# qinliuliuqin/Medical-Segmentation3d-Toolkit

Measured on AMD Instinct MI355X. Metric: patches/sec (96^3, 1-mod V-Net) train-step, higher is better.
Workload: dtype f32; 1 GPU; vnet(1,2) train step (fwd + Dice loss + bwd + fused Adam), 4 patches of 96^3 per GPU, fp32, random-init weights; global_batch=4, patch=96, parallelism=single GPU, wgrad_overlap=True, train_step_hipgraph=False, step_mode=auto, full=False

## Files before the change

### include/seg3d_hip.h

```cpp
#ifndef SEG3D_HIP_H
#define SEG3D_HIP_H

#ifdef __cplusplus
extern "C" {
#endif

#define SEG3D_ABI_VERSION 2

const char* seg3d_last_error(void);
int seg3d_abi_version(void);
const char* seg3d_target_arch(void);
int seg3d_device_count(void);

int seg3d_ncdhw_to_ndhwc(const float* in, float* out, int N, int C, long long S, void* stream);
int seg3d_ndhwc_to_ncdhw(const float* in, float* out, int N, int C, long long S, void* stream);
int seg3d_copy_channels(const float* src, float* dst, long long nvox, int C, int src_ld, int src_off, int dst_ld,
                        int dst_off, void* stream);

int seg3d_pack_weights_tapmajor(const float* w, float* wp, int A, int B, int BP, int T, long long sa, long long sb,
                                int flip, void* stream);
int seg3d_pack_weights_mfma(const float* w, float* wp, int A, int B, int T, long long sa, long long sb, int flip,
                            void* stream);
long long seg3d_packed_mfma_floats(int A, int B, int T);
typedef struct Seg3dPackJob {
// ... 41 lines not shown
int seg3d_bf16_to_f32(const void* src_bf16, float* dst, long long n, void* stream);
int seg3d_conv3d_k3_wino_supported(int N, int D, int H, int W, int Cin, int Cout);
int seg3d_conv3d_k3_wino_preferred(int N, int D, int H, int W, int Cin, int Cout);
long long seg3d_conv3d_k3_wino_stats_count(int N, int D, int H, int W, int Cin, int Cout);
int seg3d_conv3d_k3_wino_fwd(const float* x, const float* wp_wino, const float* bias, const float* addend, float* y,
                             float* stats_partial, int N, int D, int H, int W, int Cin, int Cout, void* stream);
int seg3d_conv3d_k3_wino2d_supported(int N, int D, int H, int W, int Cin, int Cout);
int seg3d_conv3d_k3_wino2d_preferred(int N, int D, int H, int W, int Cin, int Cout);
long long seg3d_conv3d_k3_wino2d_stats_count(int N, int D, int H, int W, int Cin, int Cout);
int seg3d_conv3d_k3_wino2d_fwd(const float* x, const float* wp_wino2d, const float* bias, const float* addend, float* y,
                               float* stats_partial, int N, int D, int H, int W, int Cin, int Cout, void* stream);
long long seg3d_conv3d_k3_wino2d_fwd_workspace_floats(int N, int D, int H, int W, int Cin, int Cout);
int seg3d_conv3d_k3_wino2d_fwd_ws(const float* x, const float* wp_wino2d, const float* bias, const float* addend, float* y,
                                  float* stats_partial, float* workspace, int N, int D, int H, int W, int Cin, int Cout,
                                  void* stream);
int seg3d_conv3d_k3_wino_wgrad_supported(int N, int D, int H, int W, int Cin, int Cout);
long long seg3d_conv3d_k3_wino_wgrad_workspace_floats(int N, int D, int H, int W, int Cin, int Cout);
int seg3d_conv3d_k3_wino_wgrad(const float* x, const float* dy, float* dw, float* workspace, int N, int D, int H, int W,
                               int Cin, int Cout, int accumulate, void* stream);
int seg3d_conv3d_k3_wino2d_wgrad_supported(int N, int D, int H, int W, int Cin, int Cout);
int seg3d_conv3d_k3_wino2d_wgrad_preferred(int N, int D, int H, int W, int Cin, int Cout);
long long seg3d_conv3d_k3_wino2d_wgrad_workspace_floats(int N, int D, int H, int W, int Cin, int Cout);
int seg3d_conv3d_k3_wino2d_wgrad(const float* x, const float* dy, float* dw, float* workspace, int N, int D, int H, int W,
                                 int Cin, int Cout, int accumulate, void* stream);
int seg3d_conv3d_k3_wino2d_fwd_variant(int N, int D, int H, int W, int Cin, int Cout);
int seg3d_conv3d_k3_wino2d_fwd_sk_chunks(int N, int D, int H, int W, int Cin, int Cout);
int seg3d_conv3d_k3_wino_wgrad_variant(int N, int D, int H, int W, int Cin, int Cout);
int seg3d_conv3d_k3_wino2d_wgrad_variant(int N, int D, int H, int W, int Cin, int Cout);
long long seg3d_conv3d_k3_bf16_stats_count(int N, int D, int H, int W, int Cin, int Cout);
long long seg3d_conv3d_k3_bf16_fwd_workspace_floats(int N, int D, int H, int W, int Cin, int Cout);
// ... 381 lines not shown
```

### medical-segmentation3d-toolkit_amd/csrc/conv_wino2d.hip

```cpp
#include "seg3d_common.h"
#include <type_traits>
#include <utility>
#include "seg3d_hip.h"
#include <stdint.h>

typedef float f32x16 __attribute__((ext_vector_type(16)));
typedef float f32x4 __attribute__((ext_vector_type(4)));
typedef float f32x2 __attribute__((ext_vector_type(2)));

#define W2_TS 8
#define W2_H (W2_TS + 2)
#define W2_NV (W2_H * W2_H * W2_H)
#define W2_NQ 16
#define W2_RAW 4096
#define W2_T (16 * W2_H * W2_NQ * 4)
#define W2_W (48 * 128)
#define W2_LDS_FLOATS (2 * W2_RAW + 2 * W2_T + 2 * W2_W)

__device__ __attribute__((aligned(16))) float w2_zero16[4];

typedef __attribute__((address_space(3))) float w2_lds_float;
__device__ __forceinline__ void w2_glds16(const float* src, float* lds_dst_wave_uniform) {
  const unsigned off = __builtin_amdgcn_readfirstlane((unsigned)(uintptr_t)(w2_lds_float*)lds_dst_wave_uniform);
  asm volatile("s_mov_b32 m0, %1\n\ts_nop 0\n\tglobal_load_lds_dwordx4 %0, off" : : "v"(src), "s"(off) : "memory", "m0");
// ... 96 lines not shown
  float bs[16];
#pragma unroll
  for (int r = 0; r < 16; ++r) bs[r] = __int_as_float(__builtin_amdgcn_readfirstlane(__float_as_int(bias[ub + r])));
  f32x4 b4;
#pragma unroll
  for (int r = 0; r < 4; ++r) b4[r] = kq == 0 ? bs[r] : (kq == 1 ? bs[4 + r] : (kq == 2 ? bs[8 + r] : bs[12 + r]));
  return b4;
}

template <bool BIAS, bool ADD>
__global__ __launch_bounds__(512, 1) void conv3d_k3_wino2d_kernel(const float* __restrict__ x, const float* __restrict__ wp,
                                                                      const float* __restrict__ bias, float* __restrict__ y,
                                                                      float* __restrict__ stats, int N, int D, int H, int W,
                                                                      int Cin, int Cout, int ntz, int nty, int ntx, int ncog,
                                                                      int nitems, const float* __restrict__ addend, int sk_per,
                                                                      float* __restrict__ skws) {
  extern __shared__ __attribute__((aligned(16))) float lds[];
  float* raw = lds;
  float* timg = lds + 2 * W2_RAW;
  float* wbuf = lds + 2 * W2_RAW + 2 * W2_T;
  const int tid = threadIdx.x;
  const int lane = tid & 63;
  const int wave = __builtin_amdgcn_readfirstlane(tid >> 6);
  const int zw = wave & 3, hh = wave >> 2;
  const int l16 = lane & 15, kq = lane >> 4;
  const int NSC = Cin >> 2;
  const int AB = Cin >> 3;
  const int G = gridDim.x;
  auto fdiv = [](int v, float r) { return (int)(((float)v + 0.5f) * r); };
  const float rNTX = 1.0f / (float)ntx, rNTY = 1.0f / (float)nty, rNTZ = 1.0f / (float)ntz, rNCOG = 1.0f / (float)ncog;

// ... 276 lines not shown
      ++gchunk;
#endif
    }

    int co_lane = cur_cog * 32 + 16 * hh + 4 * kq;
    int vo_q = quad_voxel(cur_n, cur_z0, cur_y0, cur_x0);
    const int stat_slot = (cur_n * (ntz * nty * ntx) + cur_tile) * ncog + cur_cog;
    const bool piece = sc_b > 0 || sc_e < NSC;
    float* obase = y;
    int oHW = H * W, oW = W, oC = Cout;
    if (piece) {
      obase = skws + (i64)(2 * sk_wg + (sc_b > 0 ? 0 : 1)) * (W2_TS * W2_TS * W2_TS * 32);
      oHW = W2_TS * W2_TS, oW = W2_TS, oC = 32;
      vo_q = ((2 * zw) * W2_TS + 2 * (l16 >> 2)) * W2_TS + 2 * (l16 & 3);
      co_lane = 16 * hh + 4 * kq;
    }
    int nco_lane = co_lane, nvo_q = vo_q;
    if (more_items) {
      decode(next_item, cur_n, cur_z0, cur_y0, cur_x0, cur_cog, cur_tile);
      nco_lane = cur_cog * 32 + 16 * hh + 4 * kq;
      nvo_q = quad_voxel(cur_n, cur_z0, cur_y0, cur_x0);
    }
    f32x2 s0p = {0.f, 0.f}, s1p = {0.f, 0.f};
    f32x2 v[2][2][2][2];
    auto out_transform = [&](int zz) __attribute__((always_inline)) {
#pragma unroll
      for (int h2 = 0; h2 < 2; ++h2) {
        f32x2 r0[4], r1[4];
#pragma unroll
        for (int px = 0; px < 4; ++px) {
          const f32x2 m0 = {acc[px][zz][2 * h2], acc[px][zz][2 * h2 + 1]}, m1 = {acc[4 + px][zz][2 * h2], acc[4 + px][zz][2 * h2 + 1]};
          const f32x2 m2 = {acc[8 + px][zz][2 * h2], acc[8 + px][zz][2 * h2 + 1]}, m3 = {acc[12 + px][zz][2 * h2], acc[12 + px][zz][2 * h2 + 1]};
// ... 453 lines not shown
}
extern "C" long long seg3d_conv3d_k3_wino2d_fwd_workspace_floats(int N, int D, int H, int W, int Cin, int Cout) {
  if (!seg3d_conv3d_k3_wino2d_supported(N, D, H, W, Cin, Cout)) return 0;
  return w2_sk_per(N, D, H, W, Cin, Cout) > 0 ? 2ll * seg3d_device_cus() * (W2_TS * W2_TS * W2_TS * 32) : 0;
}

extern "C" int seg3d_conv3d_k3_wino2d_fwd_variant(int N, int D, int H, int W, int Cin, int Cout) {
  if (!seg3d_conv3d_k3_wino2d_supported(N, D, H, W, Cin, Cout)) return 0;
  return w2_tiles(D, H, W) ? W2_TS : w2_cells_per_item(N, D, H, W, Cout);
}
extern "C" int seg3d_conv3d_k3_wino2d_fwd_sk_chunks(int N, int D, int H, int W, int Cin, int Cout) {
  if (!seg3d_conv3d_k3_wino2d_supported(N, D, H, W, Cin, Cout)) return 0;
  return w2_sk_per(N, D, H, W, Cin, Cout);
}

extern "C" int seg3d_conv3d_k3_wino2d_fwd_ws(const float* x, const float* wp, const float* bias, const float* addend, float* y,
                                             float* stats, float* workspace, int N, int D, int H, int W, int Cin, int Cout,
                                             void* stream) {
  SEG3D_REQUIRE(x && wp && y, "seg3d_conv3d_k3_wino2d_fwd: null pointer");
  SEG3D_REQUIRE(seg3d_conv3d_k3_wino2d_supported(N, D, H, W, Cin, Cout),
                "seg3d_conv3d_k3_wino2d_fwd: shape not supported (whole 4^3 cells, Cin %% 8 == 0, Cout %% 32 == 0)");
  const int ncog = Cout / 32;
  const int nitems = (int)w2_items(N, D, H, W, Cout);
  const int sk_per = workspace ? w2_sk_per(N, D, H, W, Cin, Cout) : 0;
  dim3 grid(sk_per > 0 ? (unsigned)seg3d_device_cus() : seg3d_persistent_grid(nitems), 1, 1);
  if (w2_tiles(D, H, W)) {
    static Seg3dOncePerDevice configured[4];
    if (int rc = seg3d_allow_full_lds(reinterpret_cast<const void*>(&conv3d_k3_wino2d_kernel<false, false>), configured[0], "conv3d_k3_wino2d")) return rc;
    if (int rc = seg3d_allow_full_lds(reinterpret_cast<const void*>(&conv3d_k3_wino2d_kernel<true, false>), configured[1], "conv3d_k3_wino2d")) return rc;
    if (int rc = seg3d_allow_full_lds(reinterpret_cast<const void*>(&conv3d_k3_wino2d_kernel<false, true>), configured[2], "conv3d_k3_wino2d")) return rc;
    if (int rc = seg3d_allow_full_lds(reinterpret_cast<const void*>(&conv3d_k3_wino2d_kernel<true, true>), configured[3], "conv3d_k3_wino2d")) return rc;
    const int ntz = D / W2_TS, nty = H / W2_TS, ntx = W / W2_TS;
#define W2_LAUNCH(B_, A_)                                                                                                       \
  hipLaunchKernelGGL((conv3d_k3_wino2d_kernel<B_, A_>), grid, dim3(64 * W2_NW), (size_t)W2_LDS_FLOATS * 4, (hipStream_t)stream, x, \
                     wp, bias, y, stats, N, D, H, W, Cin, Cout, ntz, nty, ntx, ncog, nitems, addend, sk_per, workspace)
    if (bias) {
      if (addend) W2_LAUNCH(true, true); else W2_LAUNCH(true, false);
    } else {
      if (addend) W2_LAUNCH(false, true); else W2_LAUNCH(false, false);
    }
#undef W2_LAUNCH
    if (sk_per > 0) {
      SEG3D_LAUNCH_CHECK("seg3d_conv3d_k3_wino2d_fwd");
      hipLaunchKernelGGL(conv3d_k3_wino2d_sk_finish_kernel, dim3(grid.x - 1), dim3(512), 0, (hipStream_t)stream, workspace, y, stats, D,
                         H, W, Cout, ntz, nty, ntx, ncog, nitems, Cin / 4, sk_per);
    }
  } else {
    static Seg3dOncePerDevice configured[8];
    if (int rc = seg3d_allow_full_lds(reinterpret_cast<const void*>(&conv3d_k3_wino2d_c4_kernel<false, false, 4>), configured[0], "conv3d_k3_wino2d_c4")) return rc;
    if (int rc = seg3d_allow_full_lds(reinterpret_cast<const void*>(&conv3d_k3_wino2d_c4_kernel<true, false, 4>), configured[1], "conv3d_k3_wino2d_c4")) return rc;
// ... 15 lines not shown
        if (addend) W2_LAUNCH(false, true, 4); else W2_LAUNCH(false, false, 4);
      }
    } else {
      if (bias) {
        if (addend) W2_LAUNCH(true, true, 2); else W2_LAUNCH(true, false, 2);
      } else {
        if (addend) W2_LAUNCH(false, true, 2); else W2_LAUNCH(false, false, 2);
      }
    }
#undef W2_LAUNCH
  }
  SEG3D_LAUNCH_CHECK("seg3d_conv3d_k3_wino2d_fwd");
  return SEG3D_OK;
}

extern "C" int seg3d_conv3d_k3_wino2d_fwd(const float* x, const float* wp, const float* bias, const float* addend, float* y,
                                          float* stats, int N, int D, int H, int W, int Cin, int Cout, void* stream) {
  return seg3d_conv3d_k3_wino2d_fwd_ws(x, wp, bias, addend, y, stats, nullptr, N, D, H, W, Cin, Cout, stream);
}

__device__ __forceinline__ int w2_mfma_row(int reg, int half) { return (reg & 3) + 8 * (reg >> 2) + 4 * half; }

#define G2_XV 216
#define G2_XS (G2_XV * 32)
#define G2_TS (16 * 24 * 32)
#define G2_YS (64 * 32)
#define G2_LDS_FLOATS (2 * G2_XS + G2_TS + 3 * G2_YS)
#define G2_XPC 27
#define G2_YPC 8
#define G2_GX 7
// ... 651 lines not shown
```

### medical-segmentation3d-toolkit_amd/segmentation3d/_engine.py

```python
import ctypes
import os

import torch

_HERE = os.path.dirname(os.path.abspath(__file__))
_PKG_ROOT = os.path.dirname(_HERE)
LIB_PATH = os.environ.get('SEG3D_HIP_LIB', os.path.join(_PKG_ROOT, 'lib', 'libseg3d_hip.so'))

_c_int, _c_ll, _c_f, _c_p = ctypes.c_int, ctypes.c_longlong, ctypes.c_float, ctypes.c_void_p


class Normalizer(ctypes.Structure):
    _fields_ = [('type', _c_int), ('mean', _c_f), ('stddev', _c_f), ('clip', _c_int), ('clip_lo', _c_f), ('clip_hi', _c_f)]


class Normalizers(ctypes.Structure):
    _fields_ = [('n', Normalizer * 8)]



class Intensity(ctypes.Structure):
    _fields_ = [('brightness', _c_f), ('contrast', _c_f), ('gamma', _c_f), ('invert', _c_int), ('sigma', _c_f)]


# ... 123 lines not shown
    'seg3d_conv3d_k3_thin_in_bf16out_fwd': (_c_int, [_c_p] * 5 + [_c_int] * 6 + [_c_p]),
    'seg3d_conv3d_k3_thin_in_persistent_stats_count': (_c_ll, [_c_int] * 4),
    'seg3d_conv3d_k3_thin_in_persistent_fwd': (_c_int, [_c_p] * 5 + [_c_int] * 7 + [_c_p]),
    'seg3d_conv3d_k3_thin_in_persistent_variant': (_c_int, [_c_int]),
    'seg3d_conv3d_k3_thin_in_persistent_workgroups': (_c_ll, [_c_int] * 5),
    'seg3d_conv3d_k3_wino_supported': (_c_int, [_c_int] * 6),
    'seg3d_conv3d_k3_wino_preferred': (_c_int, [_c_int] * 6),
    'seg3d_conv3d_k3_wino_stats_count': (_c_ll, [_c_int] * 6),
    'seg3d_conv3d_k3_wino_fwd': (_c_int, [_c_p] * 6 + [_c_int] * 6 + [_c_p]),
    'seg3d_conv3d_k3_wino2d_supported': (_c_int, [_c_int] * 6),
    'seg3d_conv3d_k3_wino2d_preferred': (_c_int, [_c_int] * 6),
    'seg3d_conv3d_k3_wino2d_stats_count': (_c_ll, [_c_int] * 6),
    'seg3d_conv3d_k3_wino2d_fwd': (_c_int, [_c_p] * 6 + [_c_int] * 6 + [_c_p]),
    'seg3d_conv3d_k3_wino2d_fwd_workspace_floats': (_c_ll, [_c_int] * 6),
    'seg3d_conv3d_k3_wino2d_fwd_ws': (_c_int, [_c_p] * 7 + [_c_int] * 6 + [_c_p]),
    'seg3d_conv3d_k3_wino2d_wgrad_supported': (_c_int, [_c_int] * 6),
    'seg3d_conv3d_k3_wino2d_wgrad_preferred': (_c_int, [_c_int] * 6),
    'seg3d_conv3d_k3_wino2d_wgrad_workspace_floats': (_c_ll, [_c_int] * 6),
    'seg3d_conv3d_k3_wino2d_wgrad': (_c_int, [_c_p] * 4 + [_c_int] * 7 + [_c_p]),
    'seg3d_conv3d_k3_wino_wgrad_supported': (_c_int, [_c_int] * 6),
    'seg3d_conv3d_k3_wino_wgrad_workspace_floats': (_c_ll, [_c_int] * 6),
    'seg3d_conv3d_k3_wino_wgrad': (_c_int, [_c_p] * 4 + [_c_int] * 7 + [_c_p]),
    'seg3d_conv3d_k3_wino2d_fwd_variant': (_c_int, [_c_int] * 6),
    'seg3d_conv3d_k3_wino2d_fwd_sk_chunks': (_c_int, [_c_int] * 6),
    'seg3d_conv3d_k3_wino_wgrad_variant': (_c_int, [_c_int] * 6),
    'seg3d_conv3d_k3_wino2d_wgrad_variant': (_c_int, [_c_int] * 6),
    'seg3d_conv3d_k3_thin_out_f32mfma_supported': (_c_int, [_c_int] * 2),
    'seg3d_thin_out_f32mfma_packed_floats': (_c_ll, [_c_int] * 2),
    'seg3d_pack_weights_thin_out_f32mfma': (_c_int, [_c_p, _c_p, _c_int, _c_int, _c_ll, _c_ll, _c_int, _c_p]),
    'seg3d_conv3d_k3_thin_out_f32mfma_tz': (_c_int, [_c_int] * 4),
# ... 188 lines not shown
```

### medical-segmentation3d-toolkit_amd/segmentation3d/_ops.py

```python
import contextlib
import ctypes
import math

import torch

from . import _engine as E
from . import _grad_sink as G

GN_EPS = 1e-5

_KINDS = {'k3': (3, 1, 27, False), 'k2s2': (2, 2, 8, False), 'k1': (1, 1, 1, False), 'convT': (2, 2, 8, True)}

FORCE_DIRECT = False
WINOGRAD = True
WINOGRAD2D = True
STREAM_K = True
_TWO_FORWARDS = 0
RELU_MASK = True


@contextlib.contextmanager
def two_forwards():
    global _TWO_FORWARDS
    _TWO_FORWARDS += 1
    try:
        yield
    finally:
        _TWO_FORWARDS -= 1

_ACT_BF16 = [False]
BF16_CONV_OUTPUT = True


# ... 197 lines not shown


def _to_f32(t):
    if t.dtype != torch.bfloat16:
        return t
    tc = t if t.is_contiguous() else t.contiguous()
    out = torch.empty(tc.shape, dtype=torch.float32, device=tc.device)
    E.call('seg3d_bf16_to_f32', E.ptr(tc), E.ptr(out), tc.numel(), E.stream_ptr())
    return out


def _use_mfma(cin, cout):
    return (not FORCE_DIRECT) and cin % 4 == 0 and cin >= 8 and cout >= 8


def _conv_k3_generic(xn, w, bias, A, B, sa, sb, flip, want_stats, addend=None, out_bf16=False):
    N, D, H, W_, Cin = xn.shape
    assert Cin == A
    thin_in16 = out_bf16 and not _is_bf16(xn) and A <= 8 and not FORCE_DIRECT and addend is None and not _use_mfma(A, B)
    if out_bf16 and not thin_in16 and not (_is_bf16(xn) and A % 16 == 0 and B % 4 == 0 and B >= 8 and not FORCE_DIRECT):
        out_bf16 = False
    y = _empty((N, D, H, W_, B), xn, torch.bfloat16 if out_bf16 else torch.float32)
    if _is_bf16(xn):
        if A % 16 == 0 and B % 4 == 0 and B >= 8 and not FORCE_DIRECT:
            wp = _pack_mfma(w, A, B, 27, sa, sb, flip, bf16=True)
            stats = None
            if want_stats:
                stats = _empty((N, E.query('seg3d_conv3d_k3_bf16_stats_count', N, D, H, W_, A, B), 2), xn)
            nws = E.query('seg3d_conv3d_k3_bf16_fwd_workspace_floats', N, D, H, W_, A, B)
            ws = _empty((nws,), xn) if nws else None
            E.call('seg3d_conv3d_k3_bf16_fwd', E.ptr(xn), E.ptr(wp), E.ptr(bias), E.ptr(addend), E.ptr(y), E.ptr(stats),
                   E.ptr(ws), N, D, H, W_, A, B, int(out_bf16), E.stream_ptr())
            return y, stats
# ... 217 lines not shown
        raise ValueError('conv weights must be contiguous')




def _addend_row_stride(t, C):
    if t.dim() != 5 or t.shape[4] != C or t.stride(4) != 1:
        return 0
    ld = t.stride(3)
    if ld < C or ld % 4 or t.stride(2) != ld * t.shape[3] or t.stride(1) != ld * t.shape[3] * t.shape[2] or \
            t.stride(0) != ld * t.shape[3] * t.shape[2] * t.shape[1]:
        return 0
    return ld


def conv_dgrad(dyn, w, kind, addend=None, want_bf16=None):
    if want_bf16 is None:
        want_bf16 = _is_bf16(dyn)
    N, D, H, W_, _ = dyn.shape
    if kind == 'k3':
        Cout, Cin = w.shape[0], w.shape[1]
        dx, _ = _conv_k3_generic(dyn, w, None, Cout, Cin, Cin * 27, 27, 1, False, addend=addend, out_bf16=want_bf16)
        return dx
    if addend is not None:
        if kind == 'k2s2':
            Cout, Cin = w.shape[0], w.shape[1]
            dy16 = _is_bf16(dyn) and _use_mfma(Cout, Cin) and Cin % 4 == 0
            ld = _addend_row_stride(addend, Cin)
            if _use_mfma(Cout, Cin) and Cin % 8 == 0 and ld and _is_bf16(addend) == dy16 and \
                    tuple(addend.shape) == (N, 2 * D, 2 * H, 2 * W_, Cin):
                if _is_bf16(dyn) and not dy16:
                    dyn = _to_f32(dyn)
                w16 = dy16 and Cout % 16 == 0
                wp = _pack_mfma(w, Cout, Cin, 8, Cin * 8, 8, bf16=w16)
                dx = _empty((N, 2 * D, 2 * H, 2 * W_, Cin), dyn, dyn.dtype)
                E.call('seg3d_convT3d_k2s2_scatter_addend', E.ptr(dyn), (2 if w16 else 1) if dy16 else 0, E.ptr(wp),
                       E.ptr(addend), ld, E.ptr(dx), N, D, H, W_, Cout, Cin, int(dy16), E.stream_ptr())
# ... 333 lines not shown
    if task != _JOIN_QUEUED_FOR[0]:
        _JOIN_QUEUED_FOR[0] = task
        torch.autograd.Variable._execution_engine.queue_callback(_join_after_backward)


def _views(*sinks):
    return tuple(None if s is None else s.view for s in sinks)


class ResidualLink(object):

    def __init__(self):
        self.grad = None


class ConvGnActFunction(torch.autograd.Function):

    @staticmethod
    def forward(ctx, x, weight, bias, gamma, beta, residual, kind, relu, eps, link_in=None, link_out=None, out_slot=None,
                no_backward=False):
        E.require_device(x, weight, bias, gamma, beta, residual)
        xn = to_ndhwc(x, allow_slice=(kind == 'k2s2' and no_backward))
        w = weight.detach()
        cout = w.shape[1] if kind == 'convT' else w.shape[0]
        want16 = BF16_CONV_OUTPUT and _out_bf16(cout) and (_is_bf16(xn) or (kind == 'k3' and xn.shape[4] <= 8))
        yn, partial = conv_forward(xn, w, None if bias is None else bias.detach(), kind, want_stats=True, out_bf16=want16)
        mean_rstd = gn_stats(yn, partial, eps)
        resn = None
        if residual is not None:
            resn = to_ndhwc(residual)
            if resn.shape != yn.shape:
                raise ValueError('residual shape {} does not match conv output {}'.format(tuple(residual.shape),
                                                                                          tuple(from_ndhwc(yn).shape)))
        C = yn.shape[4]
        mask = None
        if residual is not None and relu and not no_backward and relu_mask_usable(C) and not _is_bf16(yn) and \
# ... 26 lines not shown
        dy, dres, dgamma, dbeta, dbias = gn_backward(dn, outn, yn, mean_rstd, gamma, beta, ctx.relu,
                                                     want_dres=ctx.has_res and ctx.needs_input_grad[5],
                                                     want_dbias=ctx.has_bias, sinks=_views(sg, sbt, sb_),
                                                     dy_bf16=ctx.dy_bf16, mask=mask)
        dx = None
        addend = None
        if ctx.res_is_x and dres is not None and ctx.needs_input_grad[0]:
            addend, dres = dres, None
        elif ctx.link_out is not None and dres is not None:
            ctx.link_out.grad, dres = dres, None
        if ctx.link_in is not None and ctx.link_in.grad is not None:
            if addend is not None or not ctx.needs_input_grad[0]:
                raise RuntimeError('ResidualLink misuse: the linked unit must produce exactly one input gradient')
            addend, ctx.link_in.grad = ctx.link_in.grad, None
        if ctx.needs_input_grad[0]:
            dx = from_ndhwc(conv_dgrad(dy, w, ctx.kind, addend=addend, want_bf16=_is_bf16(xn)))
        dw = None
        if ctx.needs_input_grad[1]:
            if sw is not None:
                _wgrad_to_sink(xn, dy, ctx.w_shape, ctx.kind, sw.view)
            else:
                dw = conv_wgrad(xn, dy, ctx.w_shape, ctx.kind)
        return (dx, dw, dbias if ctx.has_bias else None, dgamma, dbeta,
                from_ndhwc(dres) if dres is not None else None, None, None, None, None, None, None, None)


def conv_gn_act(x, weight, bias, gamma, beta, residual=None, kind='k3', relu=True, eps=GN_EPS, link_in=None,
                link_out=None, out_slot=None):
    no_backward = not (torch.is_grad_enabled() and any(
        t is not None and t.requires_grad for t in (x, weight, bias, gamma, beta, residual)))
    if out_slot is not None and not no_backward:
        raise RuntimeError('out_slot (output written into a slice of another buffer) is an inference-only path: '
                           'call it under torch.no_grad()')
    return ConvGnActFunction.apply(x, weight, bias, gamma, beta, residual, kind, relu, eps, link_in, link_out, out_slot,
                                   no_backward)


class UpCatFunction(torch.autograd.Function):

    @staticmethod
    def forward(ctx, x, weight, bias, gamma, beta, skip, relu, eps, link_out=None, cat_buf=None):
        E.require_device(x, weight, bias, gamma, beta, skip)
        ctx.link_out = link_out
        xn = to_ndhwc(x)
        sn = to_ndhwc(skip, allow_slice=True)
        w = weight.detach()
        want16 = BF16_CONV_OUTPUT and _is_bf16(xn) and _is_bf16(sn) and _out_bf16(w.shape[1])
        yn, partial = conv_forward(xn, w, None if bias is None else bias.detach(), 'convT', want_stats=True, out_bf16=want16)
        if sn.shape[:4] != yn.shape[:4]:
            raise ValueError('cat: spatial shapes differ: {} vs {}'.format(tuple(from_ndhwc(yn).shape), tuple(skip.shape)))
        mean_rstd = gn_stats(yn, partial, eps)
        N, D, H, W_, Ca = yn.shape
        Cb = sn.shape[4]
        if Ca % 4 or Cb % 4:
            raise ValueError('fused up + cat needs channel counts that are multiples of 4')
        bf = _is_bf16(sn)
        if bf and (Ca % 16 or Cb % 16):
            raise ValueError('fused up + cat in bf16 mode needs channel counts that are multiples of 16')
# ... 3 lines not shown
                raise ValueError('up_cat: cat_buf must be the contiguous [N,D,H,W,Ca+Cb] buffer whose slice [..., Ca:] is `skip`')
            cat = cat_buf
            gn_apply(yn, mean_rstd, gamma.detach(), beta.detach(), None, relu, out=cat[..., :Ca])
        else:
            if not sn.is_contiguous():
                sn = sn.contiguous()
            cat = _empty((N, D, H, W_, Ca + Cb), yn, torch.bfloat16 if bf else torch.float32)
            gn_apply(yn, mean_rstd, gamma.detach(), beta.detach(), None, relu, out=cat[..., :Ca])
            k = 2 if bf else 1
            E.call('seg3d_copy_channels', E.ptr(sn), E.ptr(cat), N * D * H * W_, Cb // k, Cb // k, 0, (Ca + Cb) // k, Ca // k,
                   E.stream_ptr())
        ctx.dy_bf16 = bf and _is_bf16(xn) and xn.shape[4] % 16 == 0
        ctx.relu, ctx.has_bias, ctx.w_shape, ctx.ca = bool(relu), bias is not None, tuple(weight.shape), Ca
        ctx.sinks = (G.lookup(weight), G.lookup(bias), G.lookup(gamma), G.lookup(beta))
        ctx.save_for_backward(xn, w, gamma.detach(), beta.detach(), yn, mean_rstd)
        return from_ndhwc(cat)

    @staticmethod
    def backward(ctx, dout):
        xn, w, gamma, beta, yn, mean_rstd = ctx.saved_tensors
        dn = to_ndhwc(dout)
        sw, sb_, sg, sbt = ctx.sinks
        dy, _, dgamma, dbeta, dbias = gn_backward(dn[..., :ctx.ca], None, yn, mean_rstd, gamma, beta, ctx.relu,
                                                  want_dres=False, want_dbias=ctx.has_bias, sinks=_views(sg, sbt, sb_),
                                                  dy_bf16=ctx.dy_bf16)
        dx = from_ndhwc(conv_dgrad(dy, w, 'convT')) if ctx.needs_input_grad[0] else None
        dw = None
        if ctx.needs_input_grad[1]:
            if sw is not None:
                _wgrad_to_sink(xn, dy, ctx.w_shape, 'convT', sw.view)
            else:
                dw = conv_wgrad(xn, dy, ctx.w_shape, 'convT')
        dskip = None
        if ctx.needs_input_grad[5]:
            if ctx.link_out is not None:
                ctx.link_out.grad = dn[..., ctx.ca:]
            else:
                dskip = from_ndhwc(dn[..., ctx.ca:])
        return dx, dw, dbias if ctx.has_bias else None, dgamma, dbeta, dskip, None, None, None, None


def up_cat(x, weight, bias, gamma, beta, skip, relu=True, eps=GN_EPS, link_out=None, cat_buf=None):
    return UpCatFunction.apply(x, weight, bias, gamma, beta, skip, relu, eps, link_out, cat_buf)


class ConvFunction(torch.autograd.Function):

    @staticmethod
    def forward(ctx, x, weight, bias, kind):
        E.require_device(x, weight, bias)
        xn = to_ndhwc(x)
        w = weight.detach()
        yn, _ = conv_forward(xn, w, None if bias is None else bias.detach(), kind)
        ctx.kind, ctx.has_bias, ctx.w_shape = kind, bias is not None, tuple(weight.shape)
        ctx.sinks = (G.lookup(weight), G.lookup(bias))
        ctx.save_for_backward(xn, w)
        return from_ndhwc(yn)

# ... 593 lines not shown
```

### medical-segmentation3d-toolkit_amd/segmentation3d/network/module/conv_gn_relu3.py

```python
import torch.nn as nn

from segmentation3d.network.module.layers import attach_unit, run_unit

_UNIT = ('conv', 'gn', 'act')


def _kind(ksize, stride, padding):
    for kind, geo in (('k3', (3, 1, 1)), ('k2s2', (2, 2, 0)), ('k1', (1, 1, 0))):
        if (int(ksize), int(stride), int(padding)) == geo:
            return kind
    raise ValueError('unsupported Conv3d geometry ksize={} stride={} padding={} (the reference networks use k3/s1/p1, '
                     'k2/s2/p0 and k1)'.format(ksize, stride, padding))


class ConvGnRelu3(nn.Module):

    def __init__(self, in_channels, out_channels, ksize, stride, padding, do_act=True, bias=True):
        super(ConvGnRelu3, self).__init__()
        self.do_act = do_act
        attach_unit(self, _UNIT, _kind(ksize, stride, padding), in_channels, out_channels, act=do_act, bias=bias)

    def forward(self, input, residual=None, force_act=False, link_in=None, link_out=None, out_slot=None):
        return run_unit(self, _UNIT, input, relu=self.do_act or force_act, residual=residual, link_in=link_in,
                        link_out=link_out, out_slot=out_slot)


class BottConvGnRelu3(nn.Module):

    def __init__(self, in_channels, out_channels, ksize, stride, padding, ratio, do_act=True, bias=True):
        super(BottConvGnRelu3, self).__init__()
        narrow = in_channels // ratio
        stages = ((in_channels, narrow, True), (narrow, narrow, True), (narrow, out_channels, do_act))
        for k, (cin, cout, act) in enumerate(stages, start=1):
            setattr(self, 'conv{}'.format(k), ConvGnRelu3(cin, cout, ksize, stride, padding, do_act=act, bias=bias))

    def forward(self, input, residual=None, force_act=False, link_in=None, link_out=None, out_slot=None):
        squeezed = self.conv2(self.conv1(input, link_in=link_in))
        return self.conv3(squeezed, residual=residual, force_act=force_act, link_out=link_out, out_slot=out_slot)
```

### medical-segmentation3d-toolkit_amd/segmentation3d/network/module/residual_block3.py

```python
import torch.nn as nn

from segmentation3d import _ops

from segmentation3d.network.module.conv_gn_relu3 import ConvGnRelu3, BottConvGnRelu3
from segmentation3d.network.module.layers import ReLU


def _residual_forward(ops, input, out_slot=None):
    n = len(ops)
    if n == 1:
        return ops[0](input, residual=input, force_act=True, out_slot=out_slot)
    link = _ops.ResidualLink() if input.requires_grad else None
    output = ops[0](input, link_in=link)
    for i in range(1, n - 1):
        output = ops[i](output)
    return ops[n - 1](output, residual=input, force_act=True, link_out=link, out_slot=out_slot)


class _ResidualBase(nn.Module):

    def _build(self, make_unit, num_convs):
        self.ops = nn.Sequential(*[make_unit(i != num_convs - 1) for i in range(num_convs)])
        self.act = ReLU(inplace=True)

    def forward(self, input, out_slot=None):
        return _residual_forward(self.ops, input, out_slot)


class ResidualBlock3(_ResidualBase):

    def __init__(self, channels, ksize, stride, padding, num_convs):
        super(ResidualBlock3, self).__init__()
        self._build(lambda act: ConvGnRelu3(channels, channels, ksize, stride, padding, do_act=act), num_convs)


class BottResidualBlock3(_ResidualBase):

    def __init__(self, channels, ksize, stride, padding, ratio, num_convs):
        super(BottResidualBlock3, self).__init__()
        self._build(lambda act: BottConvGnRelu3(channels, channels, ksize, stride, padding, ratio, do_act=act), num_convs)

# ... 6 lines not shown
```

### medical-segmentation3d-toolkit_amd/segmentation3d/network/module/vnet_upblock.py

```python
import torch.nn as nn

from segmentation3d import _ops
from segmentation3d.network.module.layers import attach_unit, run_unit
from segmentation3d.network.module.residual_block3 import make_residual_block

_UP = ('up_conv', 'up_gn', 'up_act')


class UpBlock(nn.Module):

    def __init__(self, in_channels, out_channels, num_convs, compression=False, ratio=4):
        super(UpBlock, self).__init__()
        attach_unit(self, _UP, 'convT', in_channels, out_channels // 2)
        self.rblock = make_residual_block(out_channels, num_convs, compression, ratio)

    def forward(self, input, skip, skip_link=None, cat_buf=None):
        conv, gn = self.up_conv, self.up_gn
        if conv.out_channels % 4 == 0 and skip.shape[1] % 4 == 0:
            merged = _ops.up_cat(input, conv.weight, conv.bias, gn.weight, gn.bias, skip, relu=True, eps=gn.eps,
                                 link_out=skip_link, cat_buf=cat_buf)
        else:
            merged = _ops.cat_channels(run_unit(self, _UP, input, relu=True), skip)
        return self.rblock(merged)
```

Before: 288.5 patches/s.

## Store cat-gradient dgrad output as split halves to skip channel slicing copies

```diff
diff --git a/include/seg3d_hip.h b/include/seg3d_hip.h
--- a/include/seg3d_hip.h
+++ b/include/seg3d_hip.h
@@ -79,6 +79,10 @@
 int seg3d_conv3d_k3_wino2d_fwd_ws(const float* x, const float* wp_wino2d, const float* bias, const float* addend, float* y,
                                   float* stats_partial, float* workspace, int N, int D, int H, int W, int Cin, int Cout,
                                   void* stream);
+int seg3d_conv3d_k3_wino2d_split_supported(int N, int D, int H, int W, int Cin, int Cout);
+int seg3d_conv3d_k3_wino2d_fwd_split(const float* x, const float* wp_wino2d, const float* bias, const float* addend, float* y_lo,
+                                     float* y_hi, float* stats_partial, int N, int D, int H, int W, int Cin, int Cout,
+                                     void* stream);
 int seg3d_conv3d_k3_wino_wgrad_supported(int N, int D, int H, int W, int Cin, int Cout);
 long long seg3d_conv3d_k3_wino_wgrad_workspace_floats(int N, int D, int H, int W, int Cin, int Cout);
 int seg3d_conv3d_k3_wino_wgrad(const float* x, const float* dy, float* dw, float* workspace, int N, int D, int H, int W,
diff --git a/medical-segmentation3d-toolkit_amd/csrc/conv_wino2d.hip b/medical-segmentation3d-toolkit_amd/csrc/conv_wino2d.hip
--- a/medical-segmentation3d-toolkit_amd/csrc/conv_wino2d.hip
+++ b/medical-segmentation3d-toolkit_amd/csrc/conv_wino2d.hip
@@ -134,7 +134,7 @@
                                                                       float* __restrict__ stats, int N, int D, int H, int W,
                                                                       int Cin, int Cout, int ntz, int nty, int ntx, int ncog,
                                                                       int nitems, const float* __restrict__ addend, int sk_per,
-                                                                      float* __restrict__ skws) {
+                                                                      float* __restrict__ skws, float* __restrict__ y_hi) {
   extern __shared__ __attribute__((aligned(16))) float lds[];
   float* raw = lds;
   float* timg = lds + 2 * W2_RAW;
@@ -441,8 +441,12 @@
       oHW = W2_TS * W2_TS, oW = W2_TS, oC = 32;
       vo_q = ((2 * zw) * W2_TS + 2 * (l16 >> 2)) * W2_TS + 2 * (l16 & 3);
       co_lane = 16 * hh + 4 * kq;
-    }
-    int nco_lane = co_lane, nvo_q = vo_q;
+    } else if (y_hi) {
+      obase = hh ? y_hi : y;
+      oC = 16;
+      co_lane = 4 * kq;
+    }
+    int nco_lane = cur_cog * 32 + 16 * hh + 4 * kq, nvo_q = vo_q;
     if (more_items) {
       decode(next_item, cur_n, cur_z0, cur_y0, cur_x0, cur_cog, cur_tile);
       nco_lane = cur_cog * 32 + 16 * hh + 4 * kq;
@@ -926,15 +930,11 @@
   return w2_sk_per(N, D, H, W, Cin, Cout);
 }
 
-extern "C" int seg3d_conv3d_k3_wino2d_fwd_ws(const float* x, const float* wp, const float* bias, const float* addend, float* y,
-                                             float* stats, float* workspace, int N, int D, int H, int W, int Cin, int Cout,
-                                             void* stream) {
-  SEG3D_REQUIRE(x && wp && y, "seg3d_conv3d_k3_wino2d_fwd: null pointer");
-  SEG3D_REQUIRE(seg3d_conv3d_k3_wino2d_supported(N, D, H, W, Cin, Cout),
-                "seg3d_conv3d_k3_wino2d_fwd: shape not supported (whole 4^3 cells, Cin %% 8 == 0, Cout %% 32 == 0)");
+static int w2_fwd_launch(const float* x, const float* wp, const float* bias, const float* addend, float* y, float* y_hi,
+                         float* stats, float* workspace, int sk_per, int N, int D, int H, int W, int Cin, int Cout,
+                         void* stream) {
   const int ncog = Cout / 32;
   const int nitems = (int)w2_items(N, D, H, W, Cout);
-  const int sk_per = workspace ? w2_sk_per(N, D, H, W, Cin, Cout) : 0;
   dim3 grid(sk_per > 0 ? (unsigned)seg3d_device_cus() : seg3d_persistent_grid(nitems), 1, 1);
   if (w2_tiles(D, H, W)) {
     static Seg3dOncePerDevice configured[4];
@@ -945,7 +945,7 @@
     const int ntz = D / W2_TS, nty = H / W2_TS, ntx = W / W2_TS;
 #define W2_LAUNCH(B_, A_)                                                                                                       \
   hipLaunchKernelGGL((conv3d_k3_wino2d_kernel<B_, A_>), grid, dim3(64 * W2_NW), (size_t)W2_LDS_FLOATS * 4, (hipStream_t)stream, x, \
-                     wp, bias, y, stats, N, D, H, W, Cin, Cout, ntz, nty, ntx, ncog, nitems, addend, sk_per, workspace)
+                     wp, bias, y, stats, N, D, H, W, Cin, Cout, ntz, nty, ntx, ncog, nitems, addend, sk_per, workspace, y_hi)
     if (bias) {
       if (addend) W2_LAUNCH(true, true); else W2_LAUNCH(true, false);
     } else {
@@ -991,6 +991,29 @@
   return SEG3D_OK;
 }
 
+extern "C" int seg3d_conv3d_k3_wino2d_fwd_ws(const float* x, const float* wp, const float* bias, const float* addend, float* y,
+                                             float* stats, float* workspace, int N, int D, int H, int W, int Cin, int Cout,
+                                             void* stream) {
+  SEG3D_REQUIRE(x && wp && y, "seg3d_conv3d_k3_wino2d_fwd: null pointer");
+  SEG3D_REQUIRE(seg3d_conv3d_k3_wino2d_supported(N, D, H, W, Cin, Cout),
+                "seg3d_conv3d_k3_wino2d_fwd: shape not supported (whole 4^3 cells, Cin %% 8 == 0, Cout %% 32 == 0)");
+  const int sk_per = workspace ? w2_sk_per(N, D, H, W, Cin, Cout) : 0;
+  return w2_fwd_launch(x, wp, bias, addend, y, nullptr, stats, workspace, sk_per, N, D, H, W, Cin, Cout, stream);
+}
+
+extern "C" int seg3d_conv3d_k3_wino2d_split_supported(int N, int D, int H, int W, int Cin, int Cout) {
+  if (!seg3d_conv3d_k3_wino2d_supported(N, D, H, W, Cin, Cout)) return 0;
+  return w2_tiles(D, H, W) && Cout == 32;
+}
+extern "C" int seg3d_conv3d_k3_wino2d_fwd_split(const float* x, const float* wp, const float* bias, const float* addend,
+                                                float* y_lo, float* y_hi, float* stats, int N, int D, int H, int W, int Cin,
+                                                int Cout, void* stream) {
+  SEG3D_REQUIRE(x && wp && y_lo && y_hi, "seg3d_conv3d_k3_wino2d_fwd_split: null pointer");
+  SEG3D_REQUIRE(seg3d_conv3d_k3_wino2d_split_supported(N, D, H, W, Cin, Cout),
+                "seg3d_conv3d_k3_wino2d_fwd_split: shape not supported (whole 8^3 tiles, Cin %% 8 == 0, Cout == 32)");
+  return w2_fwd_launch(x, wp, bias, addend, y_lo, y_hi, stats, nullptr, 0, N, D, H, W, Cin, Cout, stream);
+}
+
 extern "C" int seg3d_conv3d_k3_wino2d_fwd(const float* x, const float* wp, const float* bias, const float* addend, float* y,
                                           float* stats, int N, int D, int H, int W, int Cin, int Cout, void* stream) {
   return seg3d_conv3d_k3_wino2d_fwd_ws(x, wp, bias, addend, y, stats, nullptr, N, D, H, W, Cin, Cout, stream);
diff --git a/medical-segmentation3d-toolkit_amd/segmentation3d/_engine.py b/medical-segmentation3d-toolkit_amd/segmentation3d/_engine.py
--- a/medical-segmentation3d-toolkit_amd/segmentation3d/_engine.py
+++ b/medical-segmentation3d-toolkit_amd/segmentation3d/_engine.py
@@ -161,6 +161,8 @@
     'seg3d_conv3d_k3_wino2d_fwd': (_c_int, [_c_p] * 6 + [_c_int] * 6 + [_c_p]),
     'seg3d_conv3d_k3_wino2d_fwd_workspace_floats': (_c_ll, [_c_int] * 6),
     'seg3d_conv3d_k3_wino2d_fwd_ws': (_c_int, [_c_p] * 7 + [_c_int] * 6 + [_c_p]),
+    'seg3d_conv3d_k3_wino2d_split_supported': (_c_int, [_c_int] * 6),
+    'seg3d_conv3d_k3_wino2d_fwd_split': (_c_int, [_c_p] * 7 + [_c_int] * 6 + [_c_p]),
     'seg3d_conv3d_k3_wino2d_wgrad_supported': (_c_int, [_c_int] * 6),
     'seg3d_conv3d_k3_wino2d_wgrad_preferred': (_c_int, [_c_int] * 6),
     'seg3d_conv3d_k3_wino2d_wgrad_workspace_floats': (_c_ll, [_c_int] * 6),
diff --git a/medical-segmentation3d-toolkit_amd/segmentation3d/_ops.py b/medical-segmentation3d-toolkit_amd/segmentation3d/_ops.py
--- a/medical-segmentation3d-toolkit_amd/segmentation3d/_ops.py
+++ b/medical-segmentation3d-toolkit_amd/segmentation3d/_ops.py
@@ -17,6 +17,7 @@
 STREAM_K = True
 _TWO_FORWARDS = 0
 RELU_MASK = True
+PLANAR_CAT_GRAD = True
 
 
 @contextlib.contextmanager
@@ -244,9 +245,26 @@
     return (not FORCE_DIRECT) and cin % 4 == 0 and cin >= 8 and cout >= 8
 
 
-def _conv_k3_generic(xn, w, bias, A, B, sa, sb, flip, want_stats, addend=None, out_bf16=False):
+def _k3_split_store(xn, A, B, out_bf16):
+    N, D, H, W_, _ = xn.shape
+    return bool(not _is_bf16(xn) and not out_bf16 and _use_mfma(A, B) and WINOGRAD and WINOGRAD2D and
+                E.query('seg3d_conv3d_k3_wino2d_preferred', N, D, H, W_, A, B) and
+                E.query('seg3d_conv3d_k3_wino2d_split_supported', N, D, H, W_, A, B) and
+                not E.query('seg3d_conv3d_k3_wino2d_fwd_sk_chunks', N, D, H, W_, A, B))
+
+
+def _conv_k3_generic(xn, w, bias, A, B, sa, sb, flip, want_stats, addend=None, out_bf16=False, split=False):
     N, D, H, W_, Cin = xn.shape
     assert Cin == A
+    if split and _k3_split_store(xn, A, B, out_bf16):
+        wp = _pack_mfma(w, A, B, 48, sa, sb, flip)
+        stats = None
+        if want_stats:
+            stats = _empty((N, E.query('seg3d_conv3d_k3_wino2d_stats_count', N, D, H, W_, A, B), 2), xn)
+        y_lo, y_hi = _empty((N, D, H, W_, 16), xn), _empty((N, D, H, W_, 16), xn)
+        E.call('seg3d_conv3d_k3_wino2d_fwd_split', E.ptr(xn), E.ptr(wp), E.ptr(bias), E.ptr(addend), E.ptr(y_lo), E.ptr(y_hi),
+               E.ptr(stats), N, D, H, W_, A, B, E.stream_ptr())
+        return (y_lo, y_hi), stats
     thin_in16 = out_bf16 and not _is_bf16(xn) and A <= 8 and not FORCE_DIRECT and addend is None and not _use_mfma(A, B)
     if out_bf16 and not thin_in16 and not (_is_bf16(xn) and A % 16 == 0 and B % 4 == 0 and B >= 8 and not FORCE_DIRECT):
         out_bf16 = False
@@ -494,13 +512,16 @@
     return ld
 
 
-def conv_dgrad(dyn, w, kind, addend=None, want_bf16=None):
+def conv_dgrad(dyn, w, kind, addend=None, want_bf16=None, split=False):
     if want_bf16 is None:
         want_bf16 = _is_bf16(dyn)
     N, D, H, W_, _ = dyn.shape
+    if split and kind != 'k3':
+        raise ValueError('conv_dgrad: only the 3x3x3 data gradient has a split store')
     if kind == 'k3':
         Cout, Cin = w.shape[0], w.shape[1]
-        dx, _ = _conv_k3_generic(dyn, w, None, Cout, Cin, Cin * 27, 27, 1, False, addend=addend, out_bf16=want_bf16)
+        dx, _ = _conv_k3_generic(dyn, w, None, Cout, Cin, Cin * 27, 27, 1, False, addend=addend, out_bf16=want_bf16,
+                                 split=split)
         return dx
     if addend is not None:
         if kind == 'k2s2':
@@ -864,12 +885,53 @@
         self.grad = None
 
 
+class CatGradSink(object):
+
+    def __init__(self):
+        self.cat_key = None
+        self.armed = False
+        self.lo = self.hi = None
+        self.token = None
+
+    def bind(self, cat):
+        if self.cat_key is not None:
+            raise RuntimeError('CatGradSink misuse: one sink serves one concatenated tensor')
+        self.cat_key = (cat.data_ptr(), tuple(cat.shape))
+
+    def arm(self, x, residual):
+        if self.cat_key is None or self.armed or residual is not x or (x.data_ptr(), tuple(x.shape)) != self.cat_key:
+            raise RuntimeError('CatGradSink misuse: the sink belongs to the one unit whose conv input AND residual are the '
+                               'concatenated tensor up_cat bound it to')
+        self.armed = True
+
+    def park(self, lo, hi, like):
+        if not self.armed or self.lo is not None:
+            raise RuntimeError('CatGradSink misuse: halves parked twice, or by a unit that did not arm the sink')
+        self.lo, self.hi = lo, hi
+        self.token = torch.empty((1,), dtype=lo.dtype, device=lo.device).expand(tuple(like.shape))
+        return self.token
+
+    def take(self, dout):
+        if self.lo is None:
+            return None
+        if dout.data_ptr() != self.token.data_ptr() or any(dout.stride()) or tuple(dout.shape) != tuple(self.token.shape):
+            raise RuntimeError('CatGradSink misuse: the concatenated tensor has another consumer besides the armed unit '
+                               '(autograd summed its gradient with the placeholder)')
+        halves, self.lo, self.hi, self.token = (self.lo, self.hi), None, None, None
+        return halves
+
+
 class ConvGnActFunction(torch.autograd.Function):
 
     @staticmethod
     def forward(ctx, x, weight, bias, gamma, beta, residual, kind, relu, eps, link_in=None, link_out=None, out_slot=None,
-                no_backward=False):
+                no_backward=False, grad_sink=None):
         E.require_device(x, weight, bias, gamma, beta, residual)
+        if grad_sink is not None:
+            if kind != 'k3' or link_in is not None:
+                raise RuntimeError('CatGradSink misuse: only a 3x3x3 unit without a ResidualLink input takes one')
+            grad_sink.arm(x, residual)
+        ctx.grad_sink = grad_sink
         xn = to_ndhwc(x, allow_slice=(kind == 'k2s2' and no_backward))
         w = weight.detach()
         cout = w.shape[1] if kind == 'convT' else w.shape[0]
@@ -926,7 +988,9 @@
                 raise RuntimeError('ResidualLink misuse: the linked unit must produce exactly one input gradient')
             addend, ctx.link_in.grad = ctx.link_in.grad, None
         if ctx.needs_input_grad[0]:
-            dx = from_ndhwc(conv_dgrad(dy, w, ctx.kind, addend=addend, want_bf16=_is_bf16(xn)))
+            split = ctx.grad_sink is not None and PLANAR_CAT_GRAD and ctx.res_is_x
+            dxn = conv_dgrad(dy, w, ctx.kind, addend=addend, want_bf16=_is_bf16(xn), split=split)
+            dx = ctx.grad_sink.park(dxn[0], dxn[1], from_ndhwc(xn)) if isinstance(dxn, tuple) else from_ndhwc(dxn)
         dw = None
         if ctx.needs_input_grad[1]:
             if sw is not None:
@@ -934,26 +998,26 @@
             else:
                 dw = conv_wgrad(xn, dy, ctx.w_shape, ctx.kind)
         return (dx, dw, dbias if ctx.has_bias else None, dgamma, dbeta,
-                from_ndhwc(dres) if dres is not None else None, None, None, None, None, None, None, None)
+                from_ndhwc(dres) if dres is not None else None, None, None, None, None, None, None, None, None)
 
 
 def conv_gn_act(x, weight, bias, gamma, beta, residual=None, kind='k3', relu=True, eps=GN_EPS, link_in=None,
-                link_out=None, out_slot=None):
+                link_out=None, out_slot=None, grad_sink=None):
     no_backward = not (torch.is_grad_enabled() and any(
         t is not None and t.requires_grad for t in (x, weight, bias, gamma, beta, residual)))
     if out_slot is not None and not no_backward:
         raise RuntimeError('out_slot (output written into a slice of another buffer) is an inference-only path: '
                            'call it under torch.no_grad()')
     return ConvGnActFunction.apply(x, weight, bias, gamma, beta, residual, kind, relu, eps, link_in, link_out, out_slot,
-                                   no_backward)
+                                   no_backward, grad_sink)
 
 
 class UpCatFunction(torch.autograd.Function):
 
     @staticmethod
-    def forward(ctx, x, weight, bias, gamma, beta, skip, relu, eps, link_out=None, cat_buf=None):
+    def forward(ctx, x, weight, bias, gamma, beta, skip, relu, eps, link_out=None, cat_buf=None, grad_sink=None):
         E.require_device(x, weight, bias, gamma, beta, skip)
-        ctx.link_out = link_out
+        ctx.link_out, ctx.grad_sink = link_out, grad_sink
         xn = to_ndhwc(x)
         sn = to_ndhwc(skip, allow_slice=True)
         w = weight.detach()
@@ -987,14 +1051,23 @@
         ctx.relu, ctx.has_bias, ctx.w_shape, ctx.ca = bool(relu), bias is not None, tuple(weight.shape), Ca
         ctx.sinks = (G.lookup(weight), G.lookup(bias), G.lookup(gamma), G.lookup(beta))
         ctx.save_for_backward(xn, w, gamma.detach(), beta.detach(), yn, mean_rstd)
+        if grad_sink is not None:
+            grad_sink.bind(from_ndhwc(cat))
         return from_ndhwc(cat)
 
     @staticmethod
     def backward(ctx, dout):
         xn, w, gamma, beta, yn, mean_rstd = ctx.saved_tensors
-        dn = to_ndhwc(dout)
+        halves = ctx.grad_sink.take(dout) if ctx.grad_sink is not None else None
+        if halves is not None:
+            d_up, d_skip = halves
+            if d_up.shape[4] != ctx.ca or tuple(d_up.shape[:4]) != tuple(yn.shape[:4]):
+                raise RuntimeError('CatGradSink misuse: the parked halves do not split the gradient at the up-branch width')
+        else:
+            dn = to_ndhwc(dout)
+            d_up, d_skip = dn[..., :ctx.ca], dn[..., ctx.ca:]
         sw, sb_, sg, sbt = ctx.sinks
-        dy, _, dgamma, dbeta, dbias = gn_backward(dn[..., :ctx.ca], None, yn, mean_rstd, gamma, beta, ctx.relu,
+        dy, _, dgamma, dbeta, dbias = gn_backward(d_up, None, yn, mean_rstd, gamma, beta, ctx.relu,
                                                   want_dres=False, want_dbias=ctx.has_bias, sinks=_views(sg, sbt, sb_),
                                                   dy_bf16=ctx.dy_bf16)
         dx = from_ndhwc(conv_dgrad(dy, w, 'convT')) if ctx.needs_input_grad[0] else None
@@ -1007,14 +1080,14 @@
         dskip = None
         if ctx.needs_input_grad[5]:
             if ctx.link_out is not None:
-                ctx.link_out.grad = dn[..., ctx.ca:]
+                ctx.link_out.grad = d_skip
             else:
-                dskip = from_ndhwc(dn[..., ctx.ca:])
-        return dx, dw, dbias if ctx.has_bias else None, dgamma, dbeta, dskip, None, None, None, None
-
-
-def up_cat(x, weight, bias, gamma, beta, skip, relu=True, eps=GN_EPS, link_out=None, cat_buf=None):
-    return UpCatFunction.apply(x, weight, bias, gamma, beta, skip, relu, eps, link_out, cat_buf)
+                dskip = from_ndhwc(d_skip)
+        return dx, dw, dbias if ctx.has_bias else None, dgamma, dbeta, dskip, None, None, None, None, None
+
+
+def up_cat(x, weight, bias, gamma, beta, skip, relu=True, eps=GN_EPS, link_out=None, cat_buf=None, grad_sink=None):
+    return UpCatFunction.apply(x, weight, bias, gamma, beta, skip, relu, eps, link_out, cat_buf, grad_sink)
 
 
 class ConvFunction(torch.autograd.Function):
diff --git a/medical-segmentation3d-toolkit_amd/segmentation3d/network/module/conv_gn_relu3.py b/medical-segmentation3d-toolkit_amd/segmentation3d/network/module/conv_gn_relu3.py
--- a/medical-segmentation3d-toolkit_amd/segmentation3d/network/module/conv_gn_relu3.py
+++ b/medical-segmentation3d-toolkit_amd/segmentation3d/network/module/conv_gn_relu3.py
@@ -20,9 +20,9 @@
         self.do_act = do_act
         attach_unit(self, _UNIT, _kind(ksize, stride, padding), in_channels, out_channels, act=do_act, bias=bias)
 
-    def forward(self, input, residual=None, force_act=False, link_in=None, link_out=None, out_slot=None):
+    def forward(self, input, residual=None, force_act=False, link_in=None, link_out=None, out_slot=None, grad_sink=None):
         return run_unit(self, _UNIT, input, relu=self.do_act or force_act, residual=residual, link_in=link_in,
-                        link_out=link_out, out_slot=out_slot)
+                        link_out=link_out, out_slot=out_slot, grad_sink=grad_sink)
 
 
 class BottConvGnRelu3(nn.Module):
diff --git a/medical-segmentation3d-toolkit_amd/segmentation3d/network/module/residual_block3.py b/medical-segmentation3d-toolkit_amd/segmentation3d/network/module/residual_block3.py
--- a/medical-segmentation3d-toolkit_amd/segmentation3d/network/module/residual_block3.py
+++ b/medical-segmentation3d-toolkit_amd/segmentation3d/network/module/residual_block3.py
@@ -6,9 +6,17 @@
 from segmentation3d.network.module.layers import ReLU
 
 
-def _residual_forward(ops, input, out_slot=None):
+def takes_cat_sink(block):
+    return isinstance(block, _ResidualBase) and len(block.ops) == 1 and isinstance(block.ops[0], ConvGnRelu3)
+
+
+def _residual_forward(ops, input, out_slot=None, cat_sink=None):
     n = len(ops)
+    if cat_sink is not None and not (n == 1 and isinstance(ops[0], ConvGnRelu3)):
+        raise RuntimeError('CatGradSink misuse: only a single-conv plain residual block takes one')
     if n == 1:
+        if cat_sink is not None:
+            return ops[0](input, residual=input, force_act=True, out_slot=out_slot, grad_sink=cat_sink)
         return ops[0](input, residual=input, force_act=True, out_slot=out_slot)
     link = _ops.ResidualLink() if input.requires_grad else None
     output = ops[0](input, link_in=link)
@@ -23,8 +31,8 @@
         self.ops = nn.Sequential(*[make_unit(i != num_convs - 1) for i in range(num_convs)])
         self.act = ReLU(inplace=True)
 
-    def forward(self, input, out_slot=None):
-        return _residual_forward(self.ops, input, out_slot)
+    def forward(self, input, out_slot=None, cat_sink=None):
+        return _residual_forward(self.ops, input, out_slot, cat_sink)
 
 
 class ResidualBlock3(_ResidualBase):
diff --git a/medical-segmentation3d-toolkit_amd/segmentation3d/network/module/vnet_upblock.py b/medical-segmentation3d-toolkit_amd/segmentation3d/network/module/vnet_upblock.py
--- a/medical-segmentation3d-toolkit_amd/segmentation3d/network/module/vnet_upblock.py
+++ b/medical-segmentation3d-toolkit_amd/segmentation3d/network/module/vnet_upblock.py
@@ -1,8 +1,9 @@
+import torch
 import torch.nn as nn
 
 from segmentation3d import _ops
 from segmentation3d.network.module.layers import attach_unit, run_unit
-from segmentation3d.network.module.residual_block3 import make_residual_block
+from segmentation3d.network.module.residual_block3 import make_residual_block, takes_cat_sink
 
 _UP = ('up_conv', 'up_gn', 'up_act')
 
@@ -17,8 +18,11 @@
     def forward(self, input, skip, skip_link=None, cat_buf=None):
         conv, gn = self.up_conv, self.up_gn
         if conv.out_channels % 4 == 0 and skip.shape[1] % 4 == 0:
+            sink = None
+            if _ops.PLANAR_CAT_GRAD and torch.is_grad_enabled() and input.requires_grad and takes_cat_sink(self.rblock):
+                sink = _ops.CatGradSink()
             merged = _ops.up_cat(input, conv.weight, conv.bias, gn.weight, gn.bias, skip, relu=True, eps=gn.eps,
-                                 link_out=skip_link, cat_buf=cat_buf)
-        else:
-            merged = _ops.cat_channels(run_unit(self, _UP, input, relu=True), skip)
+                                 link_out=skip_link, cat_buf=cat_buf, grad_sink=sink)
+            return self.rblock(merged, cat_sink=sink)
+        merged = _ops.cat_channels(run_unit(self, _UP, input, relu=True), skip)
         return self.rblock(merged)
```

After: 290.9 patches/s, median of 6. No clear change (+0.9%).
